# Haochen-Wang409/U2PL

Hardware: AMD Instinct MI355X
Metric: train images/sec at 769x769 (R101-DeepLabv3+) (higher is better)
Workload: dtype f32

## Files before the change

u2pl_amd/csrc/nn.hip:

```cpp
#include "common.h"
#include "u2pl_hip.h"

__device__ __forceinline__ float4 f4add(float4 a, float4 b) { return make_float4(a.x + b.x, a.y + b.y, a.z + b.z, a.w + b.w); }
__device__ __forceinline__ float4 f4mul(float4 a, float4 b) { return make_float4(a.x * b.x, a.y * b.y, a.z * b.z, a.w * b.w); }
__device__ __forceinline__ float4 f4sub(float4 a, float4 b) { return make_float4(a.x - b.x, a.y - b.y, a.z - b.z, a.w - b.w); }
__device__ __forceinline__ float4 f4zero() { return make_float4(0.f, 0.f, 0.f, 0.f); }

struct StatOp {
    const float* x; long ld; const float* pivot;
    __device__ __forceinline__ void get(long row, int c4, float4& v0, float4& v1) const {
        float4 v = *(const float4*)(x + row * ld + c4 * 4);
        if (pivot) v = f4sub(v, *(const float4*)(pivot + c4 * 4));
        v0 = v; v1 = f4mul(v, v);
    }
};
struct SumOp {
    const float* x; long ld;
    __device__ __forceinline__ void get(long row, int c4, float4& v0, float4& v1) const {
        v0 = *(const float4*)(x + row * ld + c4 * 4); v1 = f4zero();
    }
};
__device__ __forceinline__ float4 relu_mask_from_x(float4 g, float4 xv, const float* mean, const float* invstd, const float* gamma,
                                                   const float* beta, int c) {
    const float4 mu = *(const float4*)(mean + c), is = *(const float4*)(invstd + c), ga = *(const float4*)(gamma + c), be = *(const float4*)(beta + c);
    g.x = ((xv.x - mu.x) * is.x * ga.x + be.x) > 0.f ? g.x : 0.f;
    g.y = ((xv.y - mu.y) * is.y * ga.y + be.y) > 0.f ? g.y : 0.f;
    g.z = ((xv.z - mu.z) * is.z * ga.z + be.z) > 0.f ? g.z : 0.f;
    g.w = ((xv.w - mu.w) * is.w * ga.w + be.w) > 0.f ? g.w : 0.f;
    return g;
}
struct BnBwdOp {
    const float* dy; long lddy; const float* x; long ldx; const float* y; long ldy;
    const float* mean; const float* invstd; const float* drop; long rows_per_image; int C;
    const float* gamma; const float* relu_beta;
    __device__ __forceinline__ void get(long row, int c4, float4& v0, float4& v1) const {
        float4 g = *(const float4*)(dy + row * lddy + c4 * 4);
        float4 xv = *(const float4*)(x + row * ldx + c4 * 4);
        if (y) {
            float4 yy = *(const float4*)(y + row * ldy + c4 * 4);
            g.x = yy.x > 0.f ? g.x : 0.f; g.y = yy.y > 0.f ? g.y : 0.f;
            g.z = yy.z > 0.f ? g.z : 0.f; g.w = yy.w > 0.f ? g.w : 0.f;
        } else if (relu_beta) {
            g = relu_mask_from_x(g, xv, mean, invstd, gamma, relu_beta, c4 * 4);
        }
        if (drop) g = f4mul(g, *(const float4*)(drop + (row / rows_per_image) * C + c4 * 4));
        float4 xh = f4mul(f4sub(xv, *(const float4*)(mean + c4 * 4)), *(const float4*)(invstd + c4 * 4));
        v0 = g; v1 = f4mul(g, xh);
    }
};

template <class Op>
__global__ U2PL_HBM_KERNEL void k_colreduce_partial(Op op, long Mseg, int C, float* __restrict__ partial) {
    __shared__ float4 sh0[256], sh1[256];
    const int C4 = C >> 2;
    const int slab0 = blockIdx.z * 64;
    const int wcols = min(64, C4 - slab0);
    const int tc = wcols, tr = 256 / tc;
    const int tid = threadIdx.x, cl = tid % tc, rg = tid / tc;
    const int nblk = gridDim.x, seg = blockIdx.y;
    const long per = (Mseg + nblk - 1) / nblk;
    const long rb = seg * Mseg + blockIdx.x * per, re = min(seg * Mseg + Mseg, rb + per);
    float* out = partial + ((long)seg * nblk + blockIdx.x) * 2 * C;
    const int c4 = slab0 + cl;
    float4 a0 = f4zero(), a1 = f4zero();
    if (rg < tr) {
        float4 b0 = f4zero(), b1 = f4zero(), c0 = f4zero(), c1 = f4zero(), d0 = f4zero(), d1 = f4zero();
        long r = rb + rg;
        for (; r + 3 * (long)tr < re; r += 4 * (long)tr) {
            float4 v0, v1, w0, w1, x0, x1, y0, y1;
            op.get(r, c4, v0, v1);
            op.get(r + tr, c4, w0, w1);
            op.get(r + 2 * (long)tr, c4, x0, x1);
            op.get(r + 3 * (long)tr, c4, y0, y1);
            a0 = f4add(a0, v0); a1 = f4add(a1, v1);
            b0 = f4add(b0, w0); b1 = f4add(b1, w1);
            c0 = f4add(c0, x0); c1 = f4add(c1, x1);
            d0 = f4add(d0, y0); d1 = f4add(d1, y1);
        }
        for (; r < re; r += tr) {
            float4 v0, v1;
            op.get(r, c4, v0, v1);
            a0 = f4add(a0, v0); a1 = f4add(a1, v1);
        }
        a0 = f4add(f4add(a0, b0), f4add(c0, d0));
        a1 = f4add(f4add(a1, b1), f4add(c1, d1));
    }
    sh0[tid] = a0; sh1[tid] = a1;
    __syncthreads();
    if (rg == 0) {
        for (int k = 1; k < tr; ++k) { a0 = f4add(a0, sh0[k * tc + cl]); a1 = f4add(a1, sh1[k * tc + cl]); }
        *(float4*)(out + c4 * 4) = a0;
        *(float4*)(out + C + c4 * 4) = a1;
    }
}
__global__ __launch_bounds__(1024) void k_colreduce_final(const float* __restrict__ partial, int nblk, int C,
                                                          double* __restrict__ out) {
    __shared__ double sh[16][64];
    const int seg = blockIdx.y;
    const int cl = threadIdx.x & 63, rg = threadIdx.x >> 6;
    const int i = blockIdx.x * 64 + cl;
    double acc = 0.0;
    if (i < 2 * C) {
        const float* p = partial + (long)seg * nblk * 2 * C + i;
        int b = rg;
        for (; b + 7 * 16 < nblk; b += 8 * 16) {
            float v[8];
#pragma unroll
            for (int u = 0; u < 8; ++u) v[u] = p[(long)(b + u * 16) * 2 * C];
#pragma unroll
            for (int u = 0; u < 8; ++u) acc += (double)v[u];
        }
        for (; b < nblk; b += 16) acc += (double)p[(long)b * 2 * C];
    }
    sh[rg][cl] = acc;
    __syncthreads();
    if (rg == 0 && i < 2 * C) {
        double t = 0.0;
#pragma unroll
        for (int k = 0; k < 16; ++k) t += sh[k][cl];
        out[(long)seg * 2 * C + i] = t;
    }
}
static int colreduce_blocks(long Mseg) {
    long b = (Mseg + 63) / 64;
    return (int)(b < 1 ? 1 : (b > 512 ? 512 : b));
}
U2PL_API size_t u2pl_colreduce_workspace_bytes(long Mseg, int nseg, int C) {
    return (size_t)nseg * colreduce_blocks(Mseg) * 2 * C * sizeof(float);
}
template <class Op>
static int run_colreduce(Op op, long Mseg, int nseg, int C, void* ws, double* out, hipStream_t stream) {
    if (C % 4 || Mseg <= 0) return U2PL_EINVAL;
    const int nblk = colreduce_blocks(Mseg);
    U2PL_LAUNCH((k_colreduce_partial<Op>), dim3(nblk, nseg, cdiv(C / 4, 64)), dim3(256), 0, stream, op, Mseg, C, (float*)ws);
    U2PL_LAUNCH_CHECK();
    U2PL_LAUNCH(k_colreduce_final, dim3(cdiv(2 * C, 64), nseg), dim3(1024), 0, stream, (const float*)ws, nblk, C, out);
    U2PL_LAUNCH_CHECK();
    return 0;
}

U2PL_API int u2pl_colreduce_finish_f32(const float* partial, int nblk, int C, double* sums, hipStream_t stream) {
    U2PL_LAUNCH(k_colreduce_final, dim3(cdiv(2 * C, 64), 1), dim3(1024), 0, stream, partial, nblk, C, sums);
    U2PL_LAUNCH_CHECK();
    return 0;
}

__global__ void k_bn_stats_small(const float* __restrict__ x, long ld, int M, int C, const float* __restrict__ pivot,
                                 double* __restrict__ sums) {
    const int c = blockIdx.x * blockDim.x + threadIdx.x;
    if (c >= C) return;
    double s = 0.0;
    for (int m = 0; m < M; ++m) s += (double)x[m * ld + c];
    const double mean = s / M;
    double q = 0.0;
    for (int m = 0; m < M; ++m) { const double d = (double)x[m * ld + c] - mean; q += d * d; }
    const double dm = mean - (pivot ? (double)pivot[c] : 0.0);
    sums[c] = M * dm;
    sums[C + c] = q + M * dm * dm;
}
U2PL_API int u2pl_bn_stats_f32(const float* x, long ld, long M, int C, const float* pivot, void* workspace,
                               double* sums, hipStream_t stream) {
    if (M <= 64) {
        U2PL_LAUNCH(k_bn_stats_small, dim3(cdiv(C, 64)), dim3(64), 0, stream, x, ld, (int)M, C, pivot, sums);
        U2PL_LAUNCH_CHECK();
        return 0;
    }
    StatOp op = {x, ld, pivot};
    return run_colreduce(op, M, 1, C, workspace, sums, stream);
}
U2PL_API int u2pl_colsum_f32(const float* x, long ld, long Mseg, int nseg, int C, void* workspace, double* sums,
                             hipStream_t stream) {
    SumOp op = {x, ld};
    return run_colreduce(op, Mseg, nseg, C, workspace, sums, stream);
}
U2PL_API int u2pl_bn_bwd_sums_f32(const float* dy, long lddy, const float* x, long ldx, const float* y, long ldy,
                                  const float* mean, const float* invstd, const float* drop, long rows_per_image,
                                  long M, int C, void* workspace, double* sums, hipStream_t stream) {
    BnBwdOp op = {dy, lddy, x, ldx, y, ldy, mean, invstd, drop, rows_per_image, C, nullptr, nullptr};
    return run_colreduce(op, M, 1, C, workspace, sums, stream);
}
U2PL_API int u2pl_bn_bwd_sums_mx_f32(const float* dy, long lddy, const float* x, long ldx, const float* mean, const float* invstd,
                                     const float* gamma, const float* beta, const float* drop, long rows_per_image, long M, int C,
                                     void* workspace, double* sums, hipStream_t stream) {
    if (!gamma || !beta) return U2PL_EINVAL;
    BnBwdOp op = {dy, lddy, x, ldx, nullptr, 0, mean, invstd, drop, rows_per_image, C, gamma, beta};
    return run_colreduce(op, M, 1, C, workspace, sums, stream);
}

__global__ void k_bn_finalize(const double* __restrict__ sums, double count, const float* __restrict__ pivot, int C,
                              float eps, float momentum, float* __restrict__ mean, float* __restrict__ invstd,
                              float* __restrict__ running_mean, float* __restrict__ running_var) {
    for (int c = blockIdx.x * blockDim.x + threadIdx.x; c < C; c += gridDim.x * blockDim.x) {
        const double m1 = sums[c] / count, m2 = sums[C + c] / count;
        const double p = pivot ? (double)pivot[c] : 0.0;
        double var = m2 - m1 * m1;
        if (var < 0.0) var = 0.0;
        const double mu = p + m1;
        mean[c] = (float)mu;
        invstd[c] = (float)(1.0 / sqrt(var + (double)eps));
        if (running_mean) {
            const double unb = count > 1.0 ? var * count / (count - 1.0) : var;
            running_mean[c] = (float)((1.0 - momentum) * running_mean[c] + momentum * mu);
            running_var[c] = (float)((1.0 - momentum) * running_var[c] + momentum * unb);
        }
    }
}
U2PL_API int u2pl_bn_finalize_f32(const double* sums, double count, const float* pivot, int C, float eps,
                                  float momentum, float* mean, float* invstd, float* running_mean,
                                  float* running_var, hipStream_t stream) {
    U2PL_LAUNCH(k_bn_finalize, dim3(cdiv(C, 256)), dim3(256), 0, stream, sums, count, pivot, C, eps, momentum,
                       mean, invstd, running_mean, running_var);
    U2PL_LAUNCH_CHECK();
    return 0;
}
__global__ __launch_bounds__(1024) void k_bn_finish_finalize(const float* __restrict__ partial, int nblk, int C, double count,
                                                             const float* __restrict__ pivot, float eps, float momentum,
                                                             float* __restrict__ mean, float* __restrict__ invstd,
                                                             float* __restrict__ running_mean, float* __restrict__ running_var,
                                                             double* __restrict__ sums_out) {
    __shared__ double sh[16][64];
    __shared__ double tot[64];
    const int cl = threadIdx.x & 63, rg = threadIdx.x >> 6;
    const int c = blockIdx.x * 32 + (cl & 31);
    const int i = (cl >> 5) * C + c;
    double acc = 0.0;
    if (c < C) {
        const float* p = partial + i;
        int b = rg;
        for (; b + 7 * 16 < nblk; b += 8 * 16) {
            float v[8];
#pragma unroll
            for (int u = 0; u < 8; ++u) v[u] = p[(long)(b + u * 16) * 2 * C];
#pragma unroll
            for (int u = 0; u < 8; ++u) acc += (double)v[u];
        }
        for (; b < nblk; b += 16) acc += (double)p[(long)b * 2 * C];
    }
    sh[rg][cl] = acc;
    __syncthreads();
    if (rg == 0) {
        double t = 0.0;
#pragma unroll
        for (int k = 0; k < 16; ++k) t += sh[k][cl];
        tot[cl] = t;
        if (sums_out && c < C) sums_out[i] = t;
    }
    __syncthreads();
    if (threadIdx.x < 32 && c < C) {
        const double m1 = tot[cl] / count, m2 = tot[32 + cl] / count;
        const double pv = pivot ? (double)pivot[c] : 0.0;
        double var = m2 - m1 * m1;
        if (var < 0.0) var = 0.0;
        const double mu = pv + m1;
        mean[c] = (float)mu;
        invstd[c] = (float)(1.0 / sqrt(var + (double)eps));
        if (running_mean) {
            const double unb = count > 1.0 ? var * count / (count - 1.0) : var;
            running_mean[c] = (float)((1.0 - momentum) * running_mean[c] + momentum * mu);
            running_var[c] = (float)((1.0 - momentum) * running_var[c] + momentum * unb);
        }
    }
}
U2PL_API int u2pl_bn_finish_finalize_f32(const float* partial, int nblk, int C, double count, const float* pivot, float eps,
                                         float momentum, float* mean, float* invstd, float* running_mean, float* running_var,
                                         double* sums_out, hipStream_t stream) {
    if (!partial || nblk <= 0 || C <= 0 || !mean || !invstd) return U2PL_EINVAL;
    U2PL_LAUNCH(k_bn_finish_finalize, dim3(cdiv(C, 32)), dim3(1024), 0, stream, partial, nblk, C, count, pivot, eps, momentum, mean,
                invstd, running_mean, running_var, sums_out);
    U2PL_LAUNCH_CHECK();
    return 0;
}
__global__ void k_bn_eval_prep(const float* __restrict__ rv, int C, float eps, float* __restrict__ invstd) {
    for (int c = blockIdx.x * blockDim.x + threadIdx.x; c < C; c += gridDim.x * blockDim.x)
        invstd[c] = (float)(1.0 / sqrt((double)rv[c] + (double)eps));
}
U2PL_API int u2pl_bn_eval_invstd_f32(const float* running_var, int C, float eps, float* invstd, hipStream_t stream) {
    U2PL_LAUNCH(k_bn_eval_prep, dim3(cdiv(C, 256)), dim3(256), 0, stream, running_var, C, eps, invstd);
    U2PL_LAUNCH_CHECK();
    return 0;
}

struct EvalPrepJob { const float* rv; float* out; long long begin; int C; float eps; };
__global__ void k_bn_eval_prep_multi(const EvalPrepJob* __restrict__ jobs, int njobs, long total) {
    for (long e = blockIdx.x * (long)blockDim.x + threadIdx.x; e < total; e += (long)gridDim.x * blockDim.x) {
        int lo = 0, hi = njobs - 1;
        while (lo < hi) {
            const int mid = (lo + hi + 1) >> 1;
            if (jobs[mid].begin <= e) lo = mid; else hi = mid - 1;
        }
        const EvalPrepJob j = jobs[lo];
        const int c = (int)(e - j.begin);
        if (c < j.C) j.out[c] = (float)(1.0 / sqrt((double)j.rv[c] + (double)j.eps));
    }
}
U2PL_API size_t u2pl_bn_eval_invstd_job_bytes(void) { return sizeof(EvalPrepJob); }
U2PL_API int u2pl_bn_eval_invstd_multi_f32(const void* jobs_dev, int njobs, long total, hipStream_t stream) {
    if (njobs <= 0 || total <= 0) return 0;
    if (!jobs_dev) return U2PL_EINVAL;
    U2PL_LAUNCH(k_bn_eval_prep_multi, dim3(grid_for(total, 256)), dim3(256), 0, stream, (const EvalPrepJob*)jobs_dev, njobs, total);
    U2PL_LAUNCH_CHECK();
    return 0;
}

__global__ U2PL_HBM_KERNEL void k_bn_apply(const float* __restrict__ x, long ldx, const float* __restrict__ mean,
                           const float* __restrict__ invstd, const float* __restrict__ gamma,
                           const float* __restrict__ beta, const float* __restrict__ res, long ldr, int relu,
                           const float* __restrict__ drop, long rows_per_image, float* __restrict__ y, long ldy,
                           long M, int C, unsigned* __restrict__ y_amax) {
    const int C4 = C >> 2;
    const long total = M * C4;
    unsigned am = 0u;
    for (long i = blockIdx.x * (long)blockDim.x + threadIdx.x; i < total; i += (long)gridDim.x * blockDim.x) {
        const long r = i / C4;
        const int c = (int)(i % C4) * 4;
        float4 v = *(const float4*)(x + r * ldx + c);
        const float4 mu = *(const float4*)(mean + c), is = *(const float4*)(invstd + c);
        const float4 ga = *(const float4*)(gamma + c), be = *(const float4*)(beta + c);
        v.x = (v.x - mu.x) * is.x * ga.x + be.x; v.y = (v.y - mu.y) * is.y * ga.y + be.y;
        v.z = (v.z - mu.z) * is.z * ga.z + be.z; v.w = (v.w - mu.w) * is.w * ga.w + be.w;
        if (res) v = f4add(v, *(const float4*)(res + r * ldr + c));
        if (relu) { v.x = fmaxf(v.x, 0.f); v.y = fmaxf(v.y, 0.f); v.z = fmaxf(v.z, 0.f); v.w = fmaxf(v.w, 0.f); }
        if (drop) v = f4mul(v, *(const float4*)(drop + (r / rows_per_image) * C + c));
        *(float4*)(y + r * ldy + c) = v;
        am = amax_bits4(am, v);
    }
    if (y_amax) amax_wave_publish(am, y_amax);
}
U2PL_API int u2pl_bn_apply_f32(const float* x, long ldx, const float* mean, const float* invstd, const float* gamma,
                               const float* beta, const float* res, long ldr, int relu, const float* drop,
                               long rows_per_image, float* y, long ldy, long M, int C, hipStream_t stream) {
    if (C % 4) return U2PL_EINVAL;
    U2PL_LAUNCH(k_bn_apply, dim3(grid_for(M * (C / 4), 256)), dim3(256), 0, stream, x, ldx, mean, invstd, gamma,
                       beta, res, ldr, relu, drop, rows_per_image, y, ldy, M, C, (unsigned*)nullptr);
    U2PL_LAUNCH_CHECK();
    return 0;
}
U2PL_API int u2pl_bn_apply_amax_f32(const float* x, long ldx, const float* mean, const float* invstd, const float* gamma,
                                    const float* beta, const float* res, long ldr, int relu, const float* drop,
                                    long rows_per_image, float* y, long ldy, long M, int C, float* y_amax, hipStream_t stream) {
    if (C % 4) return U2PL_EINVAL;
    U2PL_LAUNCH(k_bn_apply, dim3(grid_for(M * (C / 4), 256)), dim3(256), 0, stream, x, ldx, mean, invstd, gamma,
                       beta, res, ldr, relu, drop, rows_per_image, y, ldy, M, C, (unsigned*)y_amax);
    U2PL_LAUNCH_CHECK();
    return 0;
}

__global__ U2PL_HBM_KERNEL void k_bn_bwd_apply(const float* __restrict__ dy, long lddy, const float* __restrict__ x, long ldx,
                               const float* __restrict__ y, long ldy, const float* __restrict__ mean,
                               const float* __restrict__ invstd, const float* __restrict__ gamma,
                               const float* __restrict__ drop, long rows_per_image,
                               const double* __restrict__ sums, double count, float* __restrict__ dx, long lddx,
                               float* __restrict__ dres, long lddr, long M, int C, const double* __restrict__ psums,
                               float* __restrict__ gsink, float* __restrict__ bsink, int accumulate,
                               unsigned* __restrict__ dx_amax, unsigned* __restrict__ dres_amax, const float* __restrict__ relu_beta) {
    unsigned am_x = 0u, am_r = 0u;
    if (psums) {
        for (long i = blockIdx.x * (long)blockDim.x + threadIdx.x; i < C; i += (long)gridDim.x * blockDim.x) {
            gsink[i] = (accumulate ? gsink[i] : 0.f) + (float)(psums[C + i] * (double)1.0f);
            bsink[i] = (accumulate ? bsink[i] : 0.f) + (float)(psums[i] * (double)1.0f);
        }
    }
    const int C4 = C >> 2;
    const long total = M * C4;
    for (long i = blockIdx.x * (long)blockDim.x + threadIdx.x; i < total; i += (long)gridDim.x * blockDim.x) {
        const long r = i / C4;
        const int c = (int)(i % C4) * 4;
        float4 g = *(const float4*)(dy + r * lddy + c);
        if (y) {
            const float4 yy = *(const float4*)(y + r * ldy + c);
            g.x = yy.x > 0.f ? g.x : 0.f; g.y = yy.y > 0.f ? g.y : 0.f;
            g.z = yy.z > 0.f ? g.z : 0.f; g.w = yy.w > 0.f ? g.w : 0.f;
        } else if (relu_beta) {
            g = relu_mask_from_x(g, *(const float4*)(x + r * ldx + c), mean, invstd, gamma, relu_beta, c);
        }
        if (drop) g = f4mul(g, *(const float4*)(drop + (r / rows_per_image) * C + c));
        if (dres) *(float4*)(dres + r * lddr + c) = g;
        am_r = amax_bits4(am_r, g);
        const float4 is = *(const float4*)(invstd + c), ga = *(const float4*)(gamma + c);
        float4 o;
        if (sums) {
            const float4 xv = *(const float4*)(x + r * ldx + c), mu = *(const float4*)(mean + c);
            const float m0x = (float)(sums[c] / count), m0y = (float)(sums[c + 1] / count);
            const float m0z = (float)(sums[c + 2] / count), m0w = (float)(sums[c + 3] / count);
            const float m1x = (float)(sums[C + c] / count), m1y = (float)(sums[C + c + 1] / count);
            const float m1z = (float)(sums[C + c + 2] / count), m1w = (float)(sums[C + c + 3] / count);
            o.x = ga.x * is.x * (g.x - m0x - (xv.x - mu.x) * is.x * m1x);
            o.y = ga.y * is.y * (g.y - m0y - (xv.y - mu.y) * is.y * m1y);
            o.z = ga.z * is.z * (g.z - m0z - (xv.z - mu.z) * is.z * m1z);
            o.w = ga.w * is.w * (g.w - m0w - (xv.w - mu.w) * is.w * m1w);
        } else {
            o = f4mul(f4mul(ga, is), g);
        }
        *(float4*)(dx + r * lddx + c) = o;
        am_x = amax_bits4(am_x, o);
    }
    if (dx_amax) amax_wave_publish(am_x, dx_amax);
    if (dres_amax) amax_wave_publish(am_r, dres_amax);
}
U2PL_API int u2pl_bn_bwd_apply_f32(const float* dy, long lddy, const float* x, long ldx, const float* y, long ldy,
                                   const float* mean, const float* invstd, const float* gamma, const float* drop,
                                   long rows_per_image, const double* sums, double count, float* dx, long lddx,
                                   float* dres, long lddr, long M, int C, hipStream_t stream) {
    if (C % 4) return U2PL_EINVAL;
    U2PL_LAUNCH(k_bn_bwd_apply, dim3(grid_for(M * (C / 4), 256)), dim3(256), 0, stream, dy, lddy, x, ldx, y, ldy,
                       mean, invstd, gamma, drop, rows_per_image, sums, count, dx, lddx, dres, lddr, M, C, (const double*)nullptr,
                       (float*)nullptr, (float*)nullptr, 0, (unsigned*)nullptr, (unsigned*)nullptr, (const float*)nullptr);
    U2PL_LAUNCH_CHECK();
    return 0;
}
U2PL_API int u2pl_bn_bwd_apply_pg_f32(const float* dy, long lddy, const float* x, long ldx, const float* y, long ldy,
                                      const float* mean, const float* invstd, const float* gamma, const float* drop,
                                      long rows_per_image, const double* sums, double count, float* dx, long lddx,
                                      float* dres, long lddr, long M, int C, const double* psums, float* gsink, float* bsink,
                                      int accumulate, hipStream_t stream) {
    if (C % 4 || !psums || !gsink || !bsink) return U2PL_EINVAL;
    U2PL_LAUNCH(k_bn_bwd_apply, dim3(grid_for(M * (C / 4), 256)), dim3(256), 0, stream, dy, lddy, x, ldx, y, ldy,
                       mean, invstd, gamma, drop, rows_per_image, sums, count, dx, lddx, dres, lddr, M, C, psums, gsink, bsink,
                       accumulate, (unsigned*)nullptr, (unsigned*)nullptr, (const float*)nullptr);
    U2PL_LAUNCH_CHECK();
    return 0;
}
U2PL_API int u2pl_bn_bwd_apply_amax_f32(const float* dy, long lddy, const float* x, long ldx, const float* y, long ldy,
                                        const float* mean, const float* invstd, const float* gamma, const float* drop,
                                        long rows_per_image, const double* sums, double count, float* dx, long lddx,
                                        float* dres, long lddr, long M, int C, const double* psums, float* gsink, float* bsink,
                                        int accumulate, float* dx_amax, float* dres_amax, const float* relu_beta, hipStream_t stream) {
    if (C % 4 || (psums && (!gsink || !bsink)) || (relu_beta && y)) return U2PL_EINVAL;
    U2PL_LAUNCH(k_bn_bwd_apply, dim3(grid_for(M * (C / 4), 256)), dim3(256), 0, stream, dy, lddy, x, ldx, y, ldy,
                       mean, invstd, gamma, drop, rows_per_image, sums, count, dx, lddx, dres, lddr, M, C, psums, gsink, bsink,
                       accumulate, (unsigned*)dx_amax, (unsigned*)dres_amax, relu_beta);
    U2PL_LAUNCH_CHECK();
    return 0;
}
__global__ void k_sums_to_f32(const double* __restrict__ s, int n, float scale, int accumulate, float* __restrict__ out) {
    for (int i = blockIdx.x * blockDim.x + threadIdx.x; i < n; i += gridDim.x * blockDim.x)
        out[i] = (accumulate ? out[i] : 0.f) + (float)(s[i] * (double)scale);
}
U2PL_API int u2pl_sums_to_f32(const double* sums, int n, float scale, int accumulate, float* out, hipStream_t stream) {
    U2PL_LAUNCH(k_sums_to_f32, dim3(cdiv(n, 256)), dim3(256), 0, stream, sums, n, scale, accumulate, out);
    U2PL_LAUNCH_CHECK();
    return 0;
}

__global__ void k_maxpool_fwd(const float* __restrict__ x, long ldx, int N, int H, int W, int C, int Ho, int Wo,
                              float* __restrict__ y, long ldy, unsigned char* __restrict__ tap) {
    const int C4 = C >> 2;
    const long total = (long)N * Ho * Wo * C4;
    for (long i = blockIdx.x * (long)blockDim.x + threadIdx.x; i < total; i += (long)gridDim.x * blockDim.x) {
        const int c = (int)(i % C4) * 4;
        long p = i / C4;
        const int wo = (int)(p % Wo);
        long t = p / Wo;
        const int ho = (int)(t % Ho), n = (int)(t / Ho);
        float4 best = make_float4(-INFINITY, -INFINITY, -INFINITY, -INFINITY);
        uchar4 bt = make_uchar4(0, 0, 0, 0);
        bool first = true;
        for (int r = 0; r < 3; ++r) {
            const int ih = ho * 2 - 1 + r;
            if (ih < 0 || ih >= H) continue;
            for (int s = 0; s < 3; ++s) {
                const int iw = wo * 2 - 1 + s;
                if (iw < 0 || iw >= W) continue;
                const float4 v = *(const float4*)(x + ((long)(n * H + ih) * W + iw) * ldx + c);
                const unsigned char k = (unsigned char)(r * 3 + s);
                if (first || v.x > best.x || v.x != v.x) { best.x = v.x; bt.x = k; }
                if (first || v.y > best.y || v.y != v.y) { best.y = v.y; bt.y = k; }
                if (first || v.z > best.z || v.z != v.z) { best.z = v.z; bt.z = k; }
                if (first || v.w > best.w || v.w != v.w) { best.w = v.w; bt.w = k; }
                first = false;
            }
        }
        *(float4*)(y + p * ldy + c) = best;
        *(uchar4*)(tap + p * C + c) = bt;
    }
}
U2PL_API int u2pl_maxpool3s2_fwd_f32(const float* x, long ldx, int N, int H, int W, int C, int Ho, int Wo, float* y,
                                     long ldy, unsigned char* tap, hipStream_t stream) {
    if (C % 4) return U2PL_EINVAL;
    U2PL_LAUNCH(k_maxpool_fwd, dim3(grid_for((long)N * Ho * Wo * (C / 4), 256)), dim3(256), 0, stream, x, ldx, N, H,
                       W, C, Ho, Wo, y, ldy, tap);
    U2PL_LAUNCH_CHECK();
    return 0;
}
__global__ void k_maxpool_bwd(const float* __restrict__ dy, long lddy, const unsigned char* __restrict__ tap, int N,
                              int H, int W, int C, int Ho, int Wo, float* __restrict__ dx, long lddx) {
    const int C4 = C >> 2;
    const long total = (long)N * H * W * C4;
    for (long i = blockIdx.x * (long)blockDim.x + threadIdx.x; i < total; i += (long)gridDim.x * blockDim.x) {
        const int c = (int)(i % C4) * 4;
        long p = i / C4;
        const int iw = (int)(p % W);
        long t = p / W;
        const int ih = (int)(t % H), n = (int)(t / H);
        float4 acc = f4zero();
        for (int ho = ih / 2; ho <= (ih + 1) / 2; ++ho) {
            if (ho >= Ho) continue;
            const int r = ih - (ho * 2 - 1);
            if (r < 0 || r > 2) continue;
            for (int wo = iw / 2; wo <= (iw + 1) / 2; ++wo) {
                if (wo >= Wo) continue;
                const int s = iw - (wo * 2 - 1);
                if (s < 0 || s > 2) continue;
                const long q = ((long)n * Ho + ho) * Wo + wo;
                const uchar4 k = *(const uchar4*)(tap + q * C + c);
                const float4 g = *(const float4*)(dy + q * lddy + c);
                const unsigned char me = (unsigned char)(r * 3 + s);
                if (k.x == me) acc.x += g.x;
                if (k.y == me) acc.y += g.y;
                if (k.z == me) acc.z += g.z;
                if (k.w == me) acc.w += g.w;
            }
        }
        *(float4*)(dx + p * lddx + c) = acc;
    }
}
U2PL_API int u2pl_maxpool3s2_bwd_f32(const float* dy, long lddy, const unsigned char* tap, int N, int H, int W, int C,
                                     int Ho, int Wo, float* dx, long lddx, hipStream_t stream) {
    U2PL_LAUNCH(k_maxpool_bwd, dim3(grid_for((long)N * H * W * (C / 4), 256)), dim3(256), 0, stream, dy, lddy, tap, N,
                       H, W, C, Ho, Wo, dx, lddx);
    U2PL_LAUNCH_CHECK();
    return 0;
}

__global__ void k_copy_rows(const float* __restrict__ src, long lds, float* __restrict__ dst, long ldd, long M, int C,
                            int accumulate) {
    const int C4 = C >> 2;
    const long total = M * C4;
    for (long i = blockIdx.x * (long)blockDim.x + threadIdx.x; i < total; i += (long)gridDim.x * blockDim.x) {
        const long r = i / C4;
        const int c = (int)(i % C4) * 4;
        float4 v = *(const float4*)(src + r * lds + c);
        if (accumulate) v = f4add(v, *(const float4*)(dst + r * ldd + c));
        *(float4*)(dst + r * ldd + c) = v;
    }
}
U2PL_API int u2pl_copy_rows_f32(const float* src, long lds, float* dst, long ldd, long M, int C, int accumulate,
                                hipStream_t stream) {
    if (C % 4) return U2PL_EINVAL;
    if (M <= 0) return 0;
    U2PL_LAUNCH(k_copy_rows, dim3(grid_for(M * (C / 4), 256)), dim3(256), 0, stream, src, lds, dst, ldd, M, C, accumulate);
    U2PL_LAUNCH_CHECK();
    return 0;
}
__global__ void k_copy_cols(const float* __restrict__ src, long lds, float* __restrict__ dst, long ldd, long M, int C) {
    const long total = M * C;
    for (long i = blockIdx.x * (long)blockDim.x + threadIdx.x; i < total; i += (long)gridDim.x * blockDim.x) {
        const long r = i / C;
        const int c = (int)(i % C);
        dst[r * ldd + c] = src[r * lds + c];
    }
}
U2PL_API int u2pl_copy_cols_f32(const float* src, long lds, float* dst, long ldd, long M, int C, hipStream_t stream) {
    if (M <= 0) return 0;
    U2PL_LAUNCH(k_copy_cols, dim3(grid_for(M * C, 256)), dim3(256), 0, stream, src, lds, dst, ldd, M, C);
    U2PL_LAUNCH_CHECK();
    return 0;
}
__global__ void k_broadcast_rows(const float* __restrict__ v, long ldv, float scale, float* __restrict__ dst, long ldd,
                                 long rows_per_image, long M, int C) {
    const int C4 = C >> 2;
    const long total = M * C4;
    for (long i = blockIdx.x * (long)blockDim.x + threadIdx.x; i < total; i += (long)gridDim.x * blockDim.x) {
        const long r = i / C4;
        const int c = (int)(i % C4) * 4;
        float4 a = *(const float4*)(v + (r / rows_per_image) * ldv + c);
        a.x *= scale; a.y *= scale; a.z *= scale; a.w *= scale;
        *(float4*)(dst + r * ldd + c) = a;
    }
}
U2PL_API int u2pl_broadcast_rows_f32(const float* v, long ldv, float scale, float* dst, long ldd, long rows_per_image,
                                     long M, int C, hipStream_t stream) {
    if (C % 4) return U2PL_EINVAL;
    U2PL_LAUNCH(k_broadcast_rows, dim3(grid_for(M * (C / 4), 256)), dim3(256), 0, stream, v, ldv, scale, dst, ldd,
                       rows_per_image, M, C);
    U2PL_LAUNCH_CHECK();
    return 0;
}

__global__ void k_bilinear_rows_fwd(const float* __restrict__ x, long ldx, int N, int h, int w, int C, int H, int W,
                                    float sy, float sx, float* __restrict__ y, long ldy) {
    const int C4 = C >> 2;
// ... 355 lines not shown
```

Before: 36.48.

## Restructure BN kernels to column-owner layout with hoisted per-channel params

BN apply and backward-apply kernels switch from a flat grid-stride over M*C/4, which needs a per-element division and reloads per-channel parameters, to a column-owner mapping. Each thread keeps its channel's parameters in registers and walks rows in unrolled groups of four, and image indices come from incremental counters instead of divisions. The column-reduce kernel gets a per-op Col object with hoisted parameters, template specialisation on mask and dropout mode, readfirstlane-based uniform row pointers, and occupancy launch bounds. The price is more register pressure, a new grid-sizing heuristic, and an EINVAL return when leading dimensions are very large.

```diff
diff --git a/u2pl_amd/csrc/nn.hip b/u2pl_amd/csrc/nn.hip
--- a/u2pl_amd/csrc/nn.hip
+++ b/u2pl_amd/csrc/nn.hip
@@ -6,51 +6,121 @@
 __device__ __forceinline__ float4 f4sub(float4 a, float4 b) { return make_float4(a.x - b.x, a.y - b.y, a.z - b.z, a.w - b.w); }
 __device__ __forceinline__ float4 f4zero() { return make_float4(0.f, 0.f, 0.f, 0.f); }
 
+template <class I>
+struct ImageOf {
+    int img; I rem, rpi, qs, ms, qj, mj;
+    __device__ __forceinline__ void init(bool on, long r, long step, long jump, long rows_per_image) {
+        img = 0; rem = 0; qs = 0; ms = 0; qj = 0; mj = 0; rpi = 1;
+        if (on) {
+            rpi = (I)rows_per_image;
+            const long q = r / rows_per_image;
+            img = (int)q; rem = (I)(r - q * rows_per_image);
+            qs = (I)(step / rows_per_image); ms = (I)(step - (step / rows_per_image) * rows_per_image);
+            qj = (I)(jump / rows_per_image); mj = (I)(jump - (jump / rows_per_image) * rows_per_image);
+        }
+    }
+    __device__ __forceinline__ void next() {
+        img += (int)qs; rem += ms;
+        if (rem >= rpi) { rem -= rpi; ++img; }
+    }
+    __device__ __forceinline__ void jump() {
+        img += (int)qj; rem += mj;
+        if (rem >= rpi) { rem -= rpi; ++img; }
+    }
+};
+typedef float f32x4 __attribute__((ext_vector_type(4)));
+__device__ __forceinline__ float4 ldg4(const U2PL_GLOBAL char* p) {
+    const f32x4 v = *(const U2PL_GLOBAL f32x4*)p;
+    return make_float4(v.x, v.y, v.z, v.w);
+}
+__device__ __forceinline__ float4 ldg4(const float* p) { return ldg4((const U2PL_GLOBAL char*)p); }
+
 struct StatOp {
     const float* x; long ld; const float* pivot;
-    __device__ __forceinline__ void get(long row, int c4, float4& v0, float4& v1) const {
-        float4 v = *(const float4*)(x + row * ld + c4 * 4);
-        if (pivot) v = f4sub(v, *(const float4*)(pivot + c4 * 4));
-        v0 = v; v1 = f4mul(v, v);
+    static constexpr int kMinWaves = 6;
+    struct Col {
+        const float* xc; long ld; float4 pv; bool shift;
+        __device__ __forceinline__ void get(long, long row, float4& v0, float4& v1) {
+            float4 v = *(const float4*)(xc + row * ld);
+            if (shift) v = f4sub(v, pv);
+            v0 = v; v1 = f4mul(v, v);
+        }
+    };
+    __device__ __forceinline__ Col col(int c4, int, long, long) const {
+        return Col{x + c4 * 4, ld, pivot ? *(const float4*)(pivot + c4 * 4) : f4zero(), pivot != nullptr};
     }
 };
 struct SumOp {
     const float* x; long ld;
-    __device__ __forceinline__ void get(long row, int c4, float4& v0, float4& v1) const {
-        v0 = *(const float4*)(x + row * ld + c4 * 4); v1 = f4zero();
-    }
+    static constexpr int kMinWaves = 6;
+    struct Col {
+        const float* xc; long ld;
+        __device__ __forceinline__ void get(long, long row, float4& v0, float4& v1) { v0 = *(const float4*)(xc + row * ld); v1 = f4zero(); }
+    };
+    __device__ __forceinline__ Col col(int c4, int, long, long) const { return Col{x + c4 * 4, ld}; }
 };
-__device__ __forceinline__ float4 relu_mask_from_x(float4 g, float4 xv, const float* mean, const float* invstd, const float* gamma,
-                                                   const float* beta, int c) {
-    const float4 mu = *(const float4*)(mean + c), is = *(const float4*)(invstd + c), ga = *(const float4*)(gamma + c), be = *(const float4*)(beta + c);
+__device__ __forceinline__ float4 relu_mask_from_x(float4 g, float4 xv, float4 mu, float4 is, float4 ga, float4 be) {
     g.x = ((xv.x - mu.x) * is.x * ga.x + be.x) > 0.f ? g.x : 0.f;
     g.y = ((xv.y - mu.y) * is.y * ga.y + be.y) > 0.f ? g.y : 0.f;
     g.z = ((xv.z - mu.z) * is.z * ga.z + be.z) > 0.f ? g.z : 0.f;
     g.w = ((xv.w - mu.w) * is.w * ga.w + be.w) > 0.f ? g.w : 0.f;
     return g;
 }
+__device__ __forceinline__ float4 relu_mask_from_y(float4 g, float4 yy) {
+    g.x = yy.x > 0.f ? g.x : 0.f; g.y = yy.y > 0.f ? g.y : 0.f;
+    g.z = yy.z > 0.f ? g.z : 0.f; g.w = yy.w > 0.f ? g.w : 0.f;
+    return g;
+}
+__device__ __forceinline__ const U2PL_GLOBAL char* uniform_global(const void* p) {
+    const unsigned long long v = (unsigned long long)p;
+    const unsigned lo = (unsigned)__builtin_amdgcn_readfirstlane((int)(unsigned)v);
+    const unsigned hi = (unsigned)__builtin_amdgcn_readfirstlane((int)(unsigned)(v >> 32));
+    return (const U2PL_GLOBAL char*)(((unsigned long long)hi << 32) | lo);
+}
+template <int MASK, bool DROP>
 struct BnBwdOp {
     const float* dy; long lddy; const float* x; long ldx; const float* y; long ldy;
     const float* mean; const float* invstd; const float* drop; long rows_per_image; int C;
     const float* gamma; const float* relu_beta;
-    __device__ __forceinline__ void get(long row, int c4, float4& v0, float4& v1) const {
-        float4 g = *(const float4*)(dy + row * lddy + c4 * 4);
-        float4 xv = *(const float4*)(x + row * ldx + c4 * 4);
-        if (y) {
-            float4 yy = *(const float4*)(y + row * ldy + c4 * 4);
-            g.x = yy.x > 0.f ? g.x : 0.f; g.y = yy.y > 0.f ? g.y : 0.f;
-            g.z = yy.z > 0.f ? g.z : 0.f; g.w = yy.w > 0.f ? g.w : 0.f;
-        } else if (relu_beta) {
-            g = relu_mask_from_x(g, xv, mean, invstd, gamma, relu_beta, c4 * 4);
-        }
-        if (drop) g = f4mul(g, *(const float4*)(drop + (row / rows_per_image) * C + c4 * 4));
-        float4 xh = f4mul(f4sub(xv, *(const float4*)(mean + c4 * 4)), *(const float4*)(invstd + c4 * 4));
-        v0 = g; v1 = f4mul(g, xh);
+    static constexpr int kMinWaves = DROP && MASK ? 5 : 6;
+    struct Col {
+        const float* dy; long lddy; const float* x; long ldx; const float* y; long ldy; const float* drop;
+        unsigned og, ox, oy; int c, C;
+        float4 mu, is, ga, be;
+        ImageOf<int> im;
+        __device__ __forceinline__ void get(long rowg, long, float4& v0, float4& v1) {
+            float4 g = ldg4(uniform_global(dy + rowg * lddy) + og);
+            const float4 xv = ldg4(uniform_global(x + rowg * ldx) + ox);
+            if (MASK == 1) g = relu_mask_from_y(g, ldg4(uniform_global(y + rowg * ldy) + oy));
+            if (MASK == 2) g = relu_mask_from_x(g, xv, mu, is, ga, be);
+            if (DROP) { g = f4mul(g, ldg4(drop + (long)im.img * C + c)); im.next(); }
+            v0 = g; v1 = f4mul(g, f4mul(f4sub(xv, mu), is));
+        }
+    };
+    __device__ __forceinline__ Col col(int c4, int rg, long r0, long step) const {
+        const int c = c4 * 4;
+        Col k;
+        k.dy = dy; k.lddy = lddy; k.x = x; k.ldx = ldx; k.y = y; k.ldy = ldy; k.drop = drop; k.c = c; k.C = C;
+        k.og = (unsigned)((rg * lddy + c) * 4); k.ox = (unsigned)((rg * ldx + c) * 4); k.oy = (unsigned)((rg * ldy + c) * 4);
+        k.mu = ldg4(mean + c); k.is = ldg4(invstd + c);
+        k.ga = MASK == 2 ? ldg4(gamma + c) : f4zero();
+        k.be = MASK == 2 ? ldg4(relu_beta + c) : f4zero();
+        k.im.init(DROP, r0, step, 0, rows_per_image);
+        return k;
     }
 };
-
+static bool bn_bwd_sums_fits(long lddy, long ldx, long ldy, const float* drop, long rows_per_image) {
+    const long lim = 1L << 21;
+    return lddy < lim && ldx < lim && ldy < lim && (!drop || (rows_per_image > 0 && rows_per_image < (1L << 30)));
+}
+
+#ifdef U2PL_HBM_MAXW
+#define U2PL_COLREDUCE_KERNEL U2PL_HBM_KERNEL
+#else
+#define U2PL_COLREDUCE_KERNEL __launch_bounds__(256, Op::kMinWaves)
+#endif
 template <class Op>
-__global__ U2PL_HBM_KERNEL void k_colreduce_partial(Op op, long Mseg, int C, float* __restrict__ partial) {
+__global__ U2PL_COLREDUCE_KERNEL void k_colreduce_partial(Op op, long Mseg, int C, float* __restrict__ partial) {
     __shared__ float4 sh0[256], sh1[256];
     const int C4 = C >> 2;
     const int slab0 = blockIdx.z * 64;
@@ -65,21 +135,18 @@
     float4 a0 = f4zero(), a1 = f4zero();
     if (rg < tr) {
         float4 b0 = f4zero(), b1 = f4zero(), c0 = f4zero(), c1 = f4zero(), d0 = f4zero(), d1 = f4zero();
-        long r = rb + rg;
-        for (; r + 3 * (long)tr < re; r += 4 * (long)tr) {
-            float4 v0, v1, w0, w1, x0, x1, y0, y1;
-            op.get(r, c4, v0, v1);
-            op.get(r + tr, c4, w0, w1);
-            op.get(r + 2 * (long)tr, c4, x0, x1);
-            op.get(r + 3 * (long)tr, c4, y0, y1);
-            a0 = f4add(a0, v0); a1 = f4add(a1, v1);
-            b0 = f4add(b0, w0); b1 = f4add(b1, w1);
-            c0 = f4add(c0, x0); c1 = f4add(c1, x1);
-            d0 = f4add(d0, y0); d1 = f4add(d1, y1);
-        }
-        for (; r < re; r += tr) {
+        long g = rb;
+        typename Op::Col col = op.col(c4, rg, g + rg, tr);
+        for (; g + rg + 3 * (long)tr < re; g += 4 * (long)tr) {
             float4 v0, v1;
-            op.get(r, c4, v0, v1);
+            col.get(g, g + rg, v0, v1);                                  a0 = f4add(a0, v0); a1 = f4add(a1, v1);
+            col.get(g + tr, g + rg + tr, v0, v1);                        b0 = f4add(b0, v0); b1 = f4add(b1, v1);
+            col.get(g + 2 * (long)tr, g + rg + 2 * (long)tr, v0, v1);    c0 = f4add(c0, v0); c1 = f4add(c1, v1);
+            col.get(g + 3 * (long)tr, g + rg + 3 * (long)tr, v0, v1);    d0 = f4add(d0, v0); d1 = f4add(d1, v1);
+        }
+        for (; g + rg < re; g += tr) {
+            float4 v0, v1;
+            col.get(g, g + rg, v0, v1);
             a0 = f4add(a0, v0); a1 = f4add(a1, v1);
         }
         a0 = f4add(f4add(a0, b0), f4add(c0, d0));
@@ -173,18 +240,29 @@
     SumOp op = {x, ld};
     return run_colreduce(op, Mseg, nseg, C, workspace, sums, stream);
 }
+template <int MASK>
+static int run_bn_bwd_sums(const float* dy, long lddy, const float* x, long ldx, const float* y, long ldy, const float* mean,
+                           const float* invstd, const float* gamma, const float* beta, const float* drop, long rows_per_image, long M,
+                           int C, void* workspace, double* sums, hipStream_t stream) {
+    if (!bn_bwd_sums_fits(lddy, ldx, ldy, drop, rows_per_image)) return U2PL_EINVAL;
+    if (drop) {
+        BnBwdOp<MASK, true> op = {dy, lddy, x, ldx, y, ldy, mean, invstd, drop, rows_per_image, C, gamma, beta};
+        return run_colreduce(op, M, 1, C, workspace, sums, stream);
+    }
+    BnBwdOp<MASK, false> op = {dy, lddy, x, ldx, y, ldy, mean, invstd, drop, rows_per_image, C, gamma, beta};
+    return run_colreduce(op, M, 1, C, workspace, sums, stream);
+}
 U2PL_API int u2pl_bn_bwd_sums_f32(const float* dy, long lddy, const float* x, long ldx, const float* y, long ldy,
                                   const float* mean, const float* invstd, const float* drop, long rows_per_image,
                                   long M, int C, void* workspace, double* sums, hipStream_t stream) {
-    BnBwdOp op = {dy, lddy, x, ldx, y, ldy, mean, invstd, drop, rows_per_image, C, nullptr, nullptr};
-    return run_colreduce(op, M, 1, C, workspace, sums, stream);
+    if (y) return run_bn_bwd_sums<1>(dy, lddy, x, ldx, y, ldy, mean, invstd, nullptr, nullptr, drop, rows_per_image, M, C, workspace, sums, stream);
+    return run_bn_bwd_sums<0>(dy, lddy, x, ldx, nullptr, 0, mean, invstd, nullptr, nullptr, drop, rows_per_image, M, C, workspace, sums, stream);
 }
 U2PL_API int u2pl_bn_bwd_sums_mx_f32(const float* dy, long lddy, const float* x, long ldx, const float* mean, const float* invstd,
                                      const float* gamma, const float* beta, const float* drop, long rows_per_image, long M, int C,
                                      void* workspace, double* sums, hipStream_t stream) {
     if (!gamma || !beta) return U2PL_EINVAL;
-    BnBwdOp op = {dy, lddy, x, ldx, nullptr, 0, mean, invstd, drop, rows_per_image, C, gamma, beta};
-    return run_colreduce(op, M, 1, C, workspace, sums, stream);
+    return run_bn_bwd_sums<2>(dy, lddy, x, ldx, nullptr, 0, mean, invstd, gamma, beta, drop, rows_per_image, M, C, workspace, sums, stream);
 }
 
 __global__ void k_bn_finalize(const double* __restrict__ sums, double count, const float* __restrict__ pivot, int C,
@@ -302,27 +380,83 @@
     return 0;
 }
 
-__global__ U2PL_HBM_KERNEL void k_bn_apply(const float* __restrict__ x, long ldx, const float* __restrict__ mean,
+#define BN_ROWS 4
+#ifdef U2PL_HBM_MAXW
+#define U2PL_BN_KERNEL(w) U2PL_HBM_KERNEL
+#else
+#define U2PL_BN_KERNEL(w) __launch_bounds__(256, w)
+#endif
+struct ColOwner { int c; bool active; long r, step, chunk; };
+__device__ __forceinline__ ColOwner col_owner(int C) {
+    const int C4 = C >> 2, slab0 = blockIdx.y * 256;
+    const int tc = min(256, C4 - slab0), tr = 256 / tc;
+    const int cl = threadIdx.x % tc, rg = threadIdx.x / tc;
+    ColOwner o;
+    o.c = (slab0 + cl) * 4; o.active = rg < tr;
+    o.step = tr; o.chunk = (long)gridDim.x * BN_ROWS * tr;
+    o.r = (long)blockIdx.x * BN_ROWS * tr + rg;
+    return o;
+}
+static dim3 bn_grid(long M, int C, int blocks_per_cu) {
+    const int C4 = C / 4, nslab = cdiv(C4, 256), tr = 256 / (C4 < 256 ? C4 : 256);
+    const int cap = 256 * blocks_per_cu / nslab;
+    return dim3(grid_for(M, BN_ROWS * tr, cap > 0 ? cap : 1), nslab);
+}
+
+template <int NR>
+__device__ __forceinline__ unsigned bn_apply_rows(const float* xp, long sx, const float* rp, long sr, float* yp, long sy,
+                                                  const float* dropc, int C, ImageOf<long>& im, int relu, float4 mu, float4 is, float4 ga,
+                                                  float4 be, unsigned am) {
+    float4 v[NR], a[NR];
+#pragma unroll
+    for (int u = 0; u < NR; ++u) v[u] = *(const float4*)(xp + u * sx);
+    if (rp) {
+#pragma unroll
+        for (int u = 0; u < NR; ++u) a[u] = *(const float4*)(rp + u * sr);
+    }
+#pragma unroll
+    for (int u = 0; u < NR; ++u) {
+        float4 t = v[u];
+        t.x = (t.x - mu.x) * is.x * ga.x + be.x; t.y = (t.y - mu.y) * is.y * ga.y + be.y;
+        t.z = (t.z - mu.z) * is.z * ga.z + be.z; t.w = (t.w - mu.w) * is.w * ga.w + be.w;
+        if (rp) t = f4add(t, a[u]);
+        if (relu) { t.x = fmaxf(t.x, 0.f); t.y = fmaxf(t.y, 0.f); t.z = fmaxf(t.z, 0.f); t.w = fmaxf(t.w, 0.f); }
+        if (dropc) { t = f4mul(t, *(const float4*)(dropc + (long)im.img * C)); im.next(); }
+        *(float4*)(yp + u * sy) = t;
+        am = amax_bits4(am, t);
+    }
+    return am;
+}
+__global__ U2PL_BN_KERNEL(6) void k_bn_apply(const float* __restrict__ x, long ldx, const float* __restrict__ mean,
                            const float* __restrict__ invstd, const float* __restrict__ gamma,
                            const float* __restrict__ beta, const float* __restrict__ res, long ldr, int relu,
                            const float* __restrict__ drop, long rows_per_image, float* __restrict__ y, long ldy,
                            long M, int C, unsigned* __restrict__ y_amax) {
-    const int C4 = C >> 2;
-    const long total = M * C4;
+    const ColOwner o = col_owner(C);
     unsigned am = 0u;
-    for (long i = blockIdx.x * (long)blockDim.x + threadIdx.x; i < total; i += (long)gridDim.x * blockDim.x) {
-        const long r = i / C4;
-        const int c = (int)(i % C4) * 4;
-        float4 v = *(const float4*)(x + r * ldx + c);
+    if (o.active) {
+        const int c = o.c;
         const float4 mu = *(const float4*)(mean + c), is = *(const float4*)(invstd + c);
         const float4 ga = *(const float4*)(gamma + c), be = *(const float4*)(beta + c);
-        v.x = (v.x - mu.x) * is.x * ga.x + be.x; v.y = (v.y - mu.y) * is.y * ga.y + be.y;
-        v.z = (v.z - mu.z) * is.z * ga.z + be.z; v.w = (v.w - mu.w) * is.w * ga.w + be.w;
-        if (res) v = f4add(v, *(const float4*)(res + r * ldr + c));
-        if (relu) { v.x = fmaxf(v.x, 0.f); v.y = fmaxf(v.y, 0.f); v.z = fmaxf(v.z, 0.f); v.w = fmaxf(v.w, 0.f); }
-        if (drop) v = f4mul(v, *(const float4*)(drop + (r / rows_per_image) * C + c));
-        *(float4*)(y + r * ldy + c) = v;
-        am = amax_bits4(am, v);
+        ImageOf<long> im;
+        im.init(drop != nullptr, o.r, o.step, o.chunk - BN_ROWS * o.step, rows_per_image);
+        const float* dropc = drop ? drop + c : nullptr;
+        const long sx = o.step * ldx, sr = o.step * ldr, sy = o.step * ldy;
+        const float* xp = x + o.r * ldx + c;
+        const float* rp = res ? res + o.r * ldr + c : nullptr;
+        float* yp = y + o.r * ldy + c;
+        for (long r = o.r; r < M; r += o.chunk) {
+            if (r + (BN_ROWS - 1) * o.step < M) {
+                am = bn_apply_rows<BN_ROWS>(xp, sx, rp, sr, yp, sy, dropc, C, im, relu, mu, is, ga, be, am);
+            } else {
+                for (int u = 0; r + u * o.step < M; ++u)
+                    am = bn_apply_rows<1>(xp + u * sx, sx, rp ? rp + u * sr : nullptr, sr, yp + u * sy, sy, dropc, C, im, relu, mu, is,
+                                          ga, be, am);
+            }
+            im.jump();
+            xp += o.chunk * ldx; yp += o.chunk * ldy;
+            if (rp) rp += o.chunk * ldr;
+        }
     }
     if (y_amax) amax_wave_publish(am, y_amax);
 }
@@ -330,7 +464,7 @@
                                const float* beta, const float* res, long ldr, int relu, const float* drop,
                                long rows_per_image, float* y, long ldy, long M, int C, hipStream_t stream) {
     if (C % 4) return U2PL_EINVAL;
-    U2PL_LAUNCH(k_bn_apply, dim3(grid_for(M * (C / 4), 256)), dim3(256), 0, stream, x, ldx, mean, invstd, gamma,
+    U2PL_LAUNCH(k_bn_apply, bn_grid(M, C, 6), dim3(256), 0, stream, x, ldx, mean, invstd, gamma,
                        beta, res, ldr, relu, drop, rows_per_image, y, ldy, M, C, (unsigned*)nullptr);
     U2PL_LAUNCH_CHECK();
     return 0;
@@ -339,13 +473,50 @@
                                     const float* beta, const float* res, long ldr, int relu, const float* drop,
                                     long rows_per_image, float* y, long ldy, long M, int C, float* y_amax, hipStream_t stream) {
     if (C % 4) return U2PL_EINVAL;
-    U2PL_LAUNCH(k_bn_apply, dim3(grid_for(M * (C / 4), 256)), dim3(256), 0, stream, x, ldx, mean, invstd, gamma,
+    U2PL_LAUNCH(k_bn_apply, bn_grid(M, C, 6), dim3(256), 0, stream, x, ldx, mean, invstd, gamma,
                        beta, res, ldr, relu, drop, rows_per_image, y, ldy, M, C, (unsigned*)y_amax);
     U2PL_LAUNCH_CHECK();
     return 0;
 }
 
-__global__ U2PL_HBM_KERNEL void k_bn_bwd_apply(const float* __restrict__ dy, long lddy, const float* __restrict__ x, long ldx,
+struct BnBwdCol { float4 mu, is, ga, be, gi, m0, m1; };
+template <int NR>
+__device__ __forceinline__ void bn_bwd_rows(const float* gp, long sg, const float* xp, long sx, const float* yp, long sy, float* dxp,
+                                            long sdx, float* drp, long sdr, const float* dropc, int C, ImageOf<long>& im, int mode,
+                                            const BnBwdCol& k, unsigned& am_x, unsigned& am_r) {
+    float4 g[NR], xv[NR], yy[NR];
+#pragma unroll
+    for (int u = 0; u < NR; ++u) g[u] = *(const float4*)(gp + u * sg);
+    if (yp) {
+#pragma unroll
+        for (int u = 0; u < NR; ++u) yy[u] = *(const float4*)(yp + u * sy);
+    }
+    if (mode) {
+#pragma unroll
+        for (int u = 0; u < NR; ++u) xv[u] = *(const float4*)(xp + u * sx);
+    }
+#pragma unroll
+    for (int u = 0; u < NR; ++u) {
+        float4 t = g[u];
+        if (yp) t = relu_mask_from_y(t, yy[u]);
+        else if (mode & 2) t = relu_mask_from_x(t, xv[u], k.mu, k.is, k.ga, k.be);
+        if (dropc) { t = f4mul(t, *(const float4*)(dropc + (long)im.img * C)); im.next(); }
+        if (drp) *(float4*)(drp + u * sdr) = t;
+        am_r = amax_bits4(am_r, t);
+        float4 o;
+        if (mode & 1) {
+            o.x = k.gi.x * (t.x - k.m0.x - (xv[u].x - k.mu.x) * k.is.x * k.m1.x);
+            o.y = k.gi.y * (t.y - k.m0.y - (xv[u].y - k.mu.y) * k.is.y * k.m1.y);
+            o.z = k.gi.z * (t.z - k.m0.z - (xv[u].z - k.mu.z) * k.is.z * k.m1.z);
+            o.w = k.gi.w * (t.w - k.m0.w - (xv[u].w - k.mu.w) * k.is.w * k.m1.w);
+        } else {
+            o = f4mul(k.gi, t);
+        }
+        *(float4*)(dxp + u * sdx) = o;
+        am_x = amax_bits4(am_x, o);
+    }
+}
+__global__ U2PL_BN_KERNEL(4) void k_bn_bwd_apply(const float* __restrict__ dy, long lddy, const float* __restrict__ x, long ldx,
                                const float* __restrict__ y, long ldy, const float* __restrict__ mean,
                                const float* __restrict__ invstd, const float* __restrict__ gamma,
                                const float* __restrict__ drop, long rows_per_image,
@@ -354,45 +525,50 @@
                                float* __restrict__ gsink, float* __restrict__ bsink, int accumulate,
                                unsigned* __restrict__ dx_amax, unsigned* __restrict__ dres_amax, const float* __restrict__ relu_beta) {
     unsigned am_x = 0u, am_r = 0u;
-    if (psums) {
+    if (psums && blockIdx.y == 0) {
         for (long i = blockIdx.x * (long)blockDim.x + threadIdx.x; i < C; i += (long)gridDim.x * blockDim.x) {
             gsink[i] = (accumulate ? gsink[i] : 0.f) + (float)(psums[C + i] * (double)1.0f);
             bsink[i] = (accumulate ? bsink[i] : 0.f) + (float)(psums[i] * (double)1.0f);
         }
     }
-    const int C4 = C >> 2;
-    const long total = M * C4;
-    for (long i = blockIdx.x * (long)blockDim.x + threadIdx.x; i < total; i += (long)gridDim.x * blockDim.x) {
-        const long r = i / C4;
-        const int c = (int)(i % C4) * 4;
-        float4 g = *(const float4*)(dy + r * lddy + c);
-        if (y) {
-            const float4 yy = *(const float4*)(y + r * ldy + c);
-            g.x = yy.x > 0.f ? g.x : 0.f; g.y = yy.y > 0.f ? g.y : 0.f;
-            g.z = yy.z > 0.f ? g.z : 0.f; g.w = yy.w > 0.f ? g.w : 0.f;
-        } else if (relu_beta) {
-            g = relu_mask_from_x(g, *(const float4*)(x + r * ldx + c), mean, invstd, gamma, relu_beta, c);
-        }
-        if (drop) g = f4mul(g, *(const float4*)(drop + (r / rows_per_image) * C + c));
-        if (dres) *(float4*)(dres + r * lddr + c) = g;
-        am_r = amax_bits4(am_r, g);
-        const float4 is = *(const float4*)(invstd + c), ga = *(const float4*)(gamma + c);
-        float4 o;
+    const ColOwner o = col_owner(C);
+    if (o.active) {
+        const int c = o.c;
+        const int mode = (sums ? 1 : 0) | (!y && relu_beta ? 2 : 0);
+        BnBwdCol k;
+        k.is = *(const float4*)(invstd + c); k.ga = *(const float4*)(gamma + c);
+        k.gi = f4mul(k.ga, k.is);
+        k.mu = mode ? *(const float4*)(mean + c) : f4zero();
+        k.be = (mode & 2) ? *(const float4*)(relu_beta + c) : f4zero();
+        k.m0 = f4zero(); k.m1 = f4zero();
         if (sums) {
-            const float4 xv = *(const float4*)(x + r * ldx + c), mu = *(const float4*)(mean + c);
-            const float m0x = (float)(sums[c] / count), m0y = (float)(sums[c + 1] / count);
-            const float m0z = (float)(sums[c + 2] / count), m0w = (float)(sums[c + 3] / count);
-            const float m1x = (float)(sums[C + c] / count), m1y = (float)(sums[C + c + 1] / count);
-            const float m1z = (float)(sums[C + c + 2] / count), m1w = (float)(sums[C + c + 3] / count);
-            o.x = ga.x * is.x * (g.x - m0x - (xv.x - mu.x) * is.x * m1x);
-            o.y = ga.y * is.y * (g.y - m0y - (xv.y - mu.y) * is.y * m1y);
-            o.z = ga.z * is.z * (g.z - m0z - (xv.z - mu.z) * is.z * m1z);
-            o.w = ga.w * is.w * (g.w - m0w - (xv.w - mu.w) * is.w * m1w);
-        } else {
-            o = f4mul(f4mul(ga, is), g);
-        }
-        *(float4*)(dx + r * lddx + c) = o;
-        am_x = amax_bits4(am_x, o);
+            k.m0 = make_float4((float)(sums[c] / count), (float)(sums[c + 1] / count), (float)(sums[c + 2] / count),
+                               (float)(sums[c + 3] / count));
+            k.m1 = make_float4((float)(sums[C + c] / count), (float)(sums[C + c + 1] / count), (float)(sums[C + c + 2] / count),
+                               (float)(sums[C + c + 3] / count));
+        }
+        ImageOf<long> im;
+        im.init(drop != nullptr, o.r, o.step, o.chunk - BN_ROWS * o.step, rows_per_image);
+        const float* dropc = drop ? drop + c : nullptr;
+        const long sg = o.step * lddy, sx = o.step * ldx, sy = o.step * ldy, sdx = o.step * lddx, sdr = o.step * lddr;
+        const float* gp = dy + o.r * lddy + c;
+        const float* xp = x + o.r * ldx + c;
+        const float* yp = y ? y + o.r * ldy + c : nullptr;
+        float* dxp = dx + o.r * lddx + c;
+        float* drp = dres ? dres + o.r * lddr + c : nullptr;
+        for (long r = o.r; r < M; r += o.chunk) {
+            if (r + (BN_ROWS - 1) * o.step < M) {
+                bn_bwd_rows<BN_ROWS>(gp, sg, xp, sx, yp, sy, dxp, sdx, drp, sdr, dropc, C, im, mode, k, am_x, am_r);
+            } else {
+                for (int u = 0; r + u * o.step < M; ++u)
+                    bn_bwd_rows<1>(gp + u * sg, sg, xp + u * sx, sx, yp ? yp + u * sy : nullptr, sy, dxp + u * sdx, sdx,
+                                   drp ? drp + u * sdr : nullptr, sdr, dropc, C, im, mode, k, am_x, am_r);
+            }
+            im.jump();
+            gp += o.chunk * lddy; xp += o.chunk * ldx; dxp += o.chunk * lddx;
+            if (yp) yp += o.chunk * ldy;
+            if (drp) drp += o.chunk * lddr;
+        }
     }
     if (dx_amax) amax_wave_publish(am_x, dx_amax);
     if (dres_amax) amax_wave_publish(am_r, dres_amax);
@@ -402,7 +578,7 @@
                                    long rows_per_image, const double* sums, double count, float* dx, long lddx,
                                    float* dres, long lddr, long M, int C, hipStream_t stream) {
     if (C % 4) return U2PL_EINVAL;
-    U2PL_LAUNCH(k_bn_bwd_apply, dim3(grid_for(M * (C / 4), 256)), dim3(256), 0, stream, dy, lddy, x, ldx, y, ldy,
+    U2PL_LAUNCH(k_bn_bwd_apply, bn_grid(M, C, 4), dim3(256), 0, stream, dy, lddy, x, ldx, y, ldy,
                        mean, invstd, gamma, drop, rows_per_image, sums, count, dx, lddx, dres, lddr, M, C, (const double*)nullptr,
                        (float*)nullptr, (float*)nullptr, 0, (unsigned*)nullptr, (unsigned*)nullptr, (const float*)nullptr);
     U2PL_LAUNCH_CHECK();
@@ -414,7 +590,7 @@
                                       float* dres, long lddr, long M, int C, const double* psums, float* gsink, float* bsink,
                                       int accumulate, hipStream_t stream) {
     if (C % 4 || !psums || !gsink || !bsink) return U2PL_EINVAL;
-    U2PL_LAUNCH(k_bn_bwd_apply, dim3(grid_for(M * (C / 4), 256)), dim3(256), 0, stream, dy, lddy, x, ldx, y, ldy,
+    U2PL_LAUNCH(k_bn_bwd_apply, bn_grid(M, C, 4), dim3(256), 0, stream, dy, lddy, x, ldx, y, ldy,
                        mean, invstd, gamma, drop, rows_per_image, sums, count, dx, lddx, dres, lddr, M, C, psums, gsink, bsink,
                        accumulate, (unsigned*)nullptr, (unsigned*)nullptr, (const float*)nullptr);
     U2PL_LAUNCH_CHECK();
@@ -426,7 +602,7 @@
                                         float* dres, long lddr, long M, int C, const double* psums, float* gsink, float* bsink,
                                         int accumulate, float* dx_amax, float* dres_amax, const float* relu_beta, hipStream_t stream) {
     if (C % 4 || (psums && (!gsink || !bsink)) || (relu_beta && y)) return U2PL_EINVAL;
-    U2PL_LAUNCH(k_bn_bwd_apply, dim3(grid_for(M * (C / 4), 256)), dim3(256), 0, stream, dy, lddy, x, ldx, y, ldy,
+    U2PL_LAUNCH(k_bn_bwd_apply, bn_grid(M, C, 4), dim3(256), 0, stream, dy, lddy, x, ldx, y, ldy,
                        mean, invstd, gamma, drop, rows_per_image, sums, count, dx, lddx, dres, lddr, M, C, psums, gsink, bsink,
                        accumulate, (unsigned*)dx_amax, (unsigned*)dres_amax, relu_beta);
     U2PL_LAUNCH_CHECK();
```

New measurement: 37.80, median of 6. +3.6%, better.
